# SEEDtk/genome.distance

Measured on AMD Instinct MI355X. Metric: genome-pair distances/sec (N×N), higher is better.
Workload: dtype u64; 1 GPU; c2: 1000 synthetic 2 Mbp genomes, DNA k=21 both strands, dictionary-rank bitsets; genomes=1000, genome_length=2000000, k=21, parallelism=rows1, dictionary_size=4000518, method=bitset

## Files before the change

### genome.distance_amd/csrc/gdist_api.hip

```cpp
#include <cstring>
#include <rocprim/rocprim.hpp>

#include <algorithm>
#include <thread>
#include <cmath>
#include <cstring>
#include <new>

#include "gdist_internal.hpp"
#include "group_stats_host.hpp"

namespace gdist {

const char* const kOptNames[OPT_COUNT] = {
#define GDIST_OPT_NAME(id, name) name,
    GDIST_OPTIONS(GDIST_OPT_NAME)
#undef GDIST_OPT_NAME
};

static int option_index(const char* name) {
    GD_REQUIRE(name != nullptr, "null option name");
    for (int i = 0; i < OPT_COUNT; i++)
        if (strcmp(kOptNames[i], name) == 0) return i;
    throw Error(GDIST_EINVAL, std::string("unknown option: ") + name);
// ... 725 lines not shown
int gdist_sets_rare_info(const gdist_sets* s, int64_t* threshold, int64_t* lists, int64_t* records) {
    return guard([&] {
        check_sets(s);
        if (threshold) *threshold = s->rare_T;
        if (lists) *lists = s->n_rare;
        if (records) *records = s->rare_records;
    });
}

int gdist_sets_sparse_info(const gdist_sets* s, int64_t* sparse_words, int64_t* dense_words, int64_t* entries) {
    return guard([&] {
        check_sets(s);
        if (sparse_words) *sparse_words = s->sparse ? s->Ws : 0;
        if (dense_words) *dense_words = s->sparse ? s->Wd : s->W;
        if (entries) *entries = s->sparse ? s->sp_entries : 0;
    });
}

int gdist_sets_variant_info(const gdist_sets* s, int64_t* kmers, int64_t* words, int64_t* entries, double* products) {
    return guard([&] {
        check_sets(s);
        if (kmers) *kmers = s->variant ? s->vw_kmers : 0;
        if (words) *words = s->variant ? s->vw_words : 0;
        if (entries) *entries = s->variant ? s->vw_entries : 0;
        if (products) *products = s->variant ? s->vw_products : 0.0;
    });
}

int gdist_sets_variant_layout(const gdist_sets* s, int* word_kmers, int* member_bytes, int64_t* row_weight_max) {
    return guard([&] {
// ... 1401 lines not shown
```

### genome.distance_amd/csrc/gdist_internal.hpp

```cpp
#pragma once

#include <hip/hip_runtime.h>
#include <rccl/rccl.h>

#include <algorithm>
#include <atomic>
#include <climits>
#include <functional>
#include <cstdint>
#include <map>
#include <memory>
#include <mutex>
#include <stdexcept>
#include <string>
#include <chrono>
#include <cstdio>
#include <cstdlib>
#include <vector>

#include "../../include/gdist.h"

namespace gdist {

struct Error : std::runtime_error {
// ... 143 lines not shown
    X(BITSET_DIAG, "bitset_diag")                        \
    X(BITSET_PARTIAL_RR, "bitset_partial_rr")     \
    X(BITSET_WG_PER_CU, "bitset_wg_per_cu")                                   \
    X(BITSET_MIN_CHUNKS, "bitset_min_chunks")      \
    X(REPS_BLOCK, "reps_block")                                \
    X(LOCUS_ORDER, "locus_order")                                            \
    X(SPARSE, "sparse")                                                                \
    X(SPARSE_ZMAX, "sparse_zmax")                    \
    X(SPARSE_WG_PER_CU, "sparse_wg_per_cu")               \
    X(SPARSE_SUN, "sparse_sun")                           \
    X(SPARSE_DYN, "sparse_dyn")                \
    X(SPARSE_BATCH, "sparse_batch")            \
    X(SPARSE_WTAIL, "sparse_wtail")            \
    X(SPARSE_DIAG22, "sparse_diag22")          \
    X(SPARSE_RPART22, "sparse_rpart22")        \
    X(SPARSE_MT, "sparse_mt")                    \
    X(SKETCH_K, "sketch_k")                                \
    X(SKETCH_TILE, "sketch_tile")                                         \
    X(SKETCH_V2, "sketch_v2")                              \
    X(SKETCH_PHASE, "sketch_phase")            \
    X(SKETCH_CAP, "sketch_cap")                          \
    X(SKETCH_RING, "sketch_ring")                              \
    X(SKETCH_WAIT, "sketch_wait")              \
    X(SPARSE_PART_BUDGET, "sparse_part_budget")        \
    X(GUIDES, "guides")                              \
    X(FORCE_EXCHANGE, "force_exchange")          \
    X(SPARSE_CHUNKS, "sparse_chunks")                         \
    X(GRAPH, "graph")                                      \
    X(TIME_KERNELS, "time_kernels")            \
    X(STEP_TIMING, "step_timing")                        \
    X(SPARSE_RARE, "sparse_rare")              \
// ... 158 lines not shown
    gdist::DevBuf post_w;
    gdist::DevBuf srare_w;
    gdist::DevBuf srare_skip;
    int64_t rare_kmers = 0;
    gdist::DevBuf guide_codes;
    gdist::DevBuf guide_keys;
    int64_t n_guide = 0;
    bool sparse = false;
    gdist::DevBuf dbits;
    gdist::DevBuf fp4;
    int64_t fp4_W = 0;
    int64_t Wd = 0;
    int64_t Ws = 0;
    gdist::DevBuf sp_off;
    gdist::DevBuf sp_ent;
    gdist::DevBuf sp_nc;
    int64_t sp_entries = 0, sp_U = 0;
    int64_t sp_pos_words = 0;
    bool sp_fold_dense = false;
    int sp_fold_slabs = 0;
    gdist::DevBuf sp_grp, sp_V, sp_T;
    int64_t sp_groups = 0, sp_group_words = 0;
    std::vector<int32_t> sp_bucket_bits;
    int64_t sp_nbk = 0;
    std::vector<double> sp_cost;
    std::vector<gdist::Summary> pack_sum;
    double sp_products = 0, sp_items = 0;
    double sp_pairs = 0;
    bool variant = false;
    int64_t vw_words = 0, vw_entries = 0, vw_kmers = 0, vw_dmin = 0, vw_max_list = 0;
// ... 410 lines not shown
```

### genome.distance_amd/csrc/sparse.hip

```cpp
#include <algorithm>
#include <map>
#include <cmath>
#include <cstring>

#include "gdist_internal.hpp"
#include "sparse_bounds.hpp"

namespace gdist {
namespace {

inline int grid_for(int64_t n, int block = 256, int64_t cap = 256 * 32) {
    int64_t g = ceil_div(n, block);
    return (int)std::max<int64_t>(1, std::min<int64_t>(g, cap));
}

constexpr int SB = 128;
constexpr int SNT = 512;
constexpr int kBucketShift = 10;

__global__ void locus_key_kernel(const uint64_t* __restrict__ gcodes, const uint64_t* __restrict__ gkeys, int64_t ng,
                                 const uint64_t* __restrict__ dict, int64_t U, uint64_t tag,
                                 uint64_t* __restrict__ key) {
    const int64_t stride = (int64_t)gridDim.x * blockDim.x;
    for (int64_t g = (int64_t)blockIdx.x * blockDim.x + threadIdx.x; g < ng; g += stride) {
// ... 293 lines not shown
    const int32_t* V = nullptr;
    const int32_t* T = nullptr;
    int m = 0;
    int64_t N = 0;
    __device__ __forceinline__ int at(int64_t i, int64_t j) const {
        if (!grp) return 0;
        const int gi = grp[i], gj = grp[j];
        int x = 0;
        if (gi >= 0) x += V[(int64_t)gi * N + j];
        if (gj >= 0) x += V[(int64_t)gj * N + i];
        if (gi >= 0 && gj >= 0) x += T[gi * m + gj];
        return x;
    }
};

__host__ __device__ __forceinline__ int cnt_index(int a, int b) {
    return ((a * 64 + ((b >> 1) ^ (a & 63))) << 1) | (b & 1);
}
__host__ __device__ __forceinline__ void cnt_pair(int t, int& a, int& b) {
    const int d = t >> 1;
    a = d >> 6;
    b = (((d & 63) ^ (a & 63)) << 1) | (t & 1);
}
__host__ __device__ __forceinline__ uint32_t row_code(int s) { return ((uint32_t)s << 8) | ((uint32_t)(s & 63) << 2); }
__host__ __device__ __forceinline__ uint32_t col_code(int s) {
    return ((uint32_t)(s & 1) << 4) | (((uint32_t)(s >> 1) << 2) << 16);
}
constexpr uint32_t kLastOfList = 32;
constexpr int kSentinelRecs = 512;
__device__ __forceinline__ void cnt_add(uint32_t* cnt, uint32_t r, uint32_t c, uint32_t v) {
    atomicAdd(reinterpret_cast<uint32_t*>(reinterpret_cast<char*>(cnt) + (r ^ (c >> 16))), v << (c & 31));
}

struct Rec3 {
    uint32_t a, b, c;
};
__device__ __forceinline__ unsigned long long rec_word(const ulonglong2& r) { return (r.x >> 32) | (r.y << 32); }
__device__ __forceinline__ uint32_t rec_row(const ulonglong2& r) { return (uint32_t)r.x; }
__device__ __forceinline__ uint32_t rec_col(const ulonglong2& r) { return (uint32_t)(r.y >> 32); }
__global__ void sparse_records_kernel(const unsigned long long* __restrict__ word, const uint8_t* __restrict__ set,
                                      int64_t n, ulonglong2* __restrict__ ent) {
    const int64_t stride = (int64_t)gridDim.x * blockDim.x;
    for (int64_t e = (int64_t)blockIdx.x * blockDim.x + threadIdx.x; e < n; e += stride) {
        const int st = set[e];
        const unsigned long long w = word[e];
        ent[e] = make_ulonglong2((unsigned long long)row_code(st) | (w << 32),
                                 (w >> 32) | ((unsigned long long)col_code(st) << 32));
    }
}

__global__ void sparse_last_kernel(const int64_t* __restrict__ off, int64_t nlists, ulonglong2* __restrict__ ent) {
    const int64_t stride = (int64_t)gridDim.x * blockDim.x;
    for (int64_t t = (int64_t)blockIdx.x * blockDim.x + threadIdx.x; t < nlists; t += stride) {
        const int64_t b = off[t], e = off[t + 1];
        if (e > b) ent[e - 1].y |= (unsigned long long)kLastOfList << 32;
    }
}

struct RareRows {
    const int64_t* soff = nullptr;
    const uint64_t* sent = nullptr;
    const uint32_t* sw = nullptr;
    const uint16_t* sskip = nullptr;
    const uint32_t* psets = nullptr;
};
inline RareRows rare_rows_of(const gdist_sets* s) {
    return RareRows{s->srare_off.as<int64_t>(), s->srare_ent.as<uint64_t>(), s->srare_w.as<uint32_t>(),
                    s->srare_skip.as<uint16_t>(), s->post_sets.as<uint32_t>()};
}

// ... 240 lines not shown
        const uint32_t v10 = (uint32_t)(__popc(a1[u].y & b0[u].y) + __popc(a1[u].z & b0[u].z)) & ne[u];
        const uint32_t v11 = (uint32_t)(__popc(a1[u].y & b1[u].y) + __popc(a1[u].z & b1[u].z)) & (ne[u] & lb);
        cnt_add(cnt, a0[u].x, b0[u].w, v00);
        cnt_add(cnt, a0[u].x, b1[u].w, v01);
        cnt_add(cnt, a1[u].x, b0[u].w, v10);
        cnt_add(cnt, a1[u].x, b1[u].w, v11);
        if (mirror) {
            cnt_add(cnt, b0[u].x, a0[u].w, v00);
            cnt_add(cnt, b1[u].x, a0[u].w, v01);
            cnt_add(cnt, b0[u].x, a1[u].w, v10);
            cnt_add(cnt, b1[u].x, a1[u].w, v11);
        }
    }
}

template <int SU, int MODE>
__device__ __forceinline__ void sparse_step(const int4* __restrict__ rec, const unsigned long long* __restrict__ masks,
                                            int W0, int last, int fb, int lane, const SparseWalk& e,
                                            uint32_t* __restrict__ cnt, bool mirror) {
    if (MODE == 0) sparse_diag_slots<SU>(rec, masks, W0, last, fb, lane, e, cnt, mirror);
    else if (MODE == 1) sparse_off_slots<SU>(rec, masks, W0, last, fb, lane, e, cnt);
    else if (MODE == 2) sparse_off22_slots<SU>(rec, masks, W0, last, fb, lane, e, cnt);
    else sparse_diag22_slots<SU>(rec, masks, W0, last, fb, lane, e, cnt, mirror);
}

template <int SUN, int MODE>
__device__ __forceinline__ void sparse_walk(const int4* __restrict__ rec, unsigned long long* __restrict__ masks,
                                            int last, int total, int lane, const SparseWalk& e,
                                            uint32_t* __restrict__ cnt, bool mirror, bool wtail) {
    constexpr int G = kWinGroups / SUN * SUN;
    for (int W0 = 0; W0 < total; W0 += 64 * G) {
        if (lane < G) masks[lane] = 0ull;
        __builtin_amdgcn_wave_barrier();
        __atomic_signal_fence(__ATOMIC_SEQ_CST);
        const uint32_t rel = (uint32_t)(last - W0);
        if (rel < 64u * G) atomicOr(&masks[rel >> 6], 1ull << (rel & 63));
        __builtin_amdgcn_wave_barrier();
// ... 11 lines not shown
        __atomic_signal_fence(__ATOMIC_SEQ_CST);
    }
}

struct TileWalk {
    const uint32_t* offA;
    const uint32_t* offB;
    const ulonglong2* ent;
    uint32_t ra0, cb0;
    uint32_t zA, zB;
    SparseWalk e;
    int rlo, rhi;
    bool rpart, diag, mirror, r22;
    bool d22;
    bool wtail;
};

template <int SUN, int MT>
__device__ __forceinline__ void global_batch(const TileWalk& tc, int64_t s0, int64_t be, int only, int lane,
                                             int4* __restrict__ wrec, unsigned long long* __restrict__ masks,
                                             uint32_t* __restrict__ cnt) {
    const uint32_t* offA = tc.offA;
    const uint32_t* offB = tc.offB;
    const ulonglong2* ent = tc.ent;
    const uint32_t ra0 = tc.ra0, cb0 = tc.cb0;
    const uint32_t zA = tc.zA, zB = tc.zB;
    const SparseWalk& e = tc.e;
    const int rlo = tc.rlo, rhi = tc.rhi;
    const bool rpart = tc.rpart, diag = tc.diag, mirror = tc.mirror, r22 = tc.r22;
    const bool d22 = MT == 2 && tc.d22;
    const bool wtail = tc.wtail;
    const int bn = be - s0 < kBatchWords ? (int)(be - s0) : kBatchWords;
    uint32_t rb = ra0, cb = cb0;
    if (lane <= bn) {
        rb = offA[2 * (s0 + lane)];
        cb = offB[2 * (s0 + lane)];
    }
    const uint32_t re = wave_next_lane(rb), ce = wave_next_lane(cb);
    int nr = 0, ncl = 0;
    if (lane < bn && (only < 0 || lane == only)) {
        nr = (int)(re - rb);
        ncl = (int)(ce - cb);
        if (rpart) {
            int a = 0, en = nr;
            for (int t = 0; t < nr; t++) {
                const int st = (int)((uint32_t)ent[(int64_t)rb + t].x >> 8);
                a += st < rlo;
                en -= st >= rhi;
            }
            rb += a;
            nr = en > a ? en - a : 0;
        }
    }
    const int ncd = diag ? ncl : (ncl + 1) >> 1;
    const int hp = (nr + 1) >> 1;
    const int P = diag ? (d22 ? (nr >= 2 ? hp * (hp + 1) / 2 : 0) : nr * (nr - 1) / 2)
                       : (r22 ? hp : nr) * ncd;
    const int incl = wave_scan_incl(P);
    const int total = __builtin_amdgcn_readlane(incl, 63);
    const unsigned long long nz = __ballot(P > 0);
    const int k = (int)__builtin_amdgcn_mbcnt_hi((uint32_t)(nz >> 32), __builtin_amdgcn_mbcnt_lo((uint32_t)nz, 0u));
    if (P > 0) {
        if (diag) {
            wrec[k] = make_int4(-(incl - P), (int32_t)(rb - ra0), 0, 0);
        } else {
            const uint32_t rcp = (uint32_t)__float_as_int(__builtin_amdgcn_rcpf(2.0f * (float)ncd));
            wrec[k] = make_int4(-2 * (incl - P), (int32_t)((rb - ra0) << 4), (int32_t)((cb - cb0) << 4),
                                (int32_t)((rcp & 0xFFFFFF00u) | (uint32_t)(2 * ncd)));
        }
    }
    if (lane == 0) {
        const int nw = __popcll(nz);
        wrec[nw] = diag ? make_int4(-total, (int32_t)zA, 0, 0)
                        : make_int4(-2 * total, (int32_t)(zA << 4), (int32_t)(zB << 4), 0);
    }
    const int last = P > 0 ? incl - 1 : 0x7FFFFFFF;
    __builtin_amdgcn_wave_barrier();
    __atomic_signal_fence(__ATOMIC_SEQ_CST);
    if (MT == 2 && diag && d22) sparse_walk<2, 3>(wrec, masks, last, total, lane, e, cnt, mirror, wtail);
    else if (diag) sparse_walk<SUN, 0>(wrec, masks, last, total, lane, e, cnt, mirror, wtail);
    else if (MT == 2 && r22) sparse_walk<MT == 2 ? SUN : 1, 2>(wrec, masks, last, total, lane, e, cnt, false, wtail);
    else sparse_walk<SUN, 1>(wrec, masks, last, total, lane, e, cnt, false, wtail);
}

template <int SUN, int MT>
__global__ __launch_bounds__(SNT, 8) void sparse_tile_kernel(
    const int64_t* __restrict__ off, const ulonglong2* __restrict__ ent, const int32_t* __restrict__ nc, int64_t Us,
    int64_t Ws, const int2* __restrict__ tiles, const int32_t* __restrict__ cbnd, const int4* __restrict__ tinfo,
    const int2* __restrict__ wgmap, int nchunks, int64_t r0, int64_t r1,
    int64_t c0, int64_t c1, int upper, int32_t* __restrict__ I, int64_t ldI, int32_t* __restrict__ part, int64_t Wdp,
    int64_t N, const unsigned long long* __restrict__ slab_bits, int slabs, GroupPart gp, int xmap, int ntiles,
    RareSlab rs, int dyn, int diag22, int rpart22, int batch, int wtail) {
    __shared__ __attribute__((aligned(16))) uint32_t cnt[SB * SB / 2];
    __shared__ int4 rec[SNW][64];
    int& next_batch = rec[0][63].w;
    const unsigned ntw = gridDim.x - (unsigned)rs.nrare;
    if (blockIdx.x >= ntw) {
        rare_slab_row(rs, (int)(blockIdx.x - ntw), r0, c0, c1, upper, cnt);
        return;
    }
    const unsigned bid = blockIdx.x;
    int tile, ch;
    if (wgmap) {
        const int2 m = wgmap[bid];
        tile = m.x;
        ch = m.y;
    } else if (xmap) {
// ... 9 lines not shown
    const int4 ti = tinfo[tile];
    cbnd += ti.x;
    const int rlo = (int)(r0 - A * SB > 0 ? r0 - A * SB : 0);
    const int rhi = (int)(r1 - A * SB < SB ? r1 - A * SB : SB);
    const bool rpart = rlo > 0 || (rhi < SB && r1 < N);
    const bool diag = A == B && !rpart, mirror = diag && !upper;
    const bool r22 = MT == 2 && !diag && (!rpart || rpart22);
    static_assert(SB * SB / 8 % SNT == 0, "whole 16-byte stores per thread");
#pragma unroll
    for (int t = 0; t < SB * SB / 8 / SNT; t++)
        reinterpret_cast<uint4*>(cnt)[t * SNT + threadIdx.x] = make_uint4(0, 0, 0, 0);
    if (threadIdx.x == 0) next_batch = SNW;
    __syncthreads();
    const int wv = __builtin_amdgcn_readfirstlane(threadIdx.x >> 6), lane = threadIdx.x & 63;
    const int64_t sb = cbnd[ch], se = cbnd[ch + 1];
    const int64_t* offA = off + A * Ws;
    const int64_t* offB = off + B * Ws;
    const int64_t ra0 = offA[sb], cb0 = offB[sb];
    const int64_t ntot = off[(int64_t)ceil_div(N, SB) * Ws];
    const uint32_t zA = (uint32_t)(ntot - ra0), zB = (uint32_t)(ntot - cb0);
    const TileWalk tc{reinterpret_cast<const uint32_t*>(offA), reinterpret_cast<const uint32_t*>(offB), ent,
                      (uint32_t)ra0, (uint32_t)cb0, zA, zB,
                      SparseWalk{reinterpret_cast<const char*>(ent + ra0), reinterpret_cast<const char*>(ent + cb0)},
                      rlo, rhi, rpart, diag, mirror, r22, diag22 != 0, wtail != 0};
    int4* wrec = &rec[wv][0];
    unsigned long long* masks = reinterpret_cast<unsigned long long*>(&rec[wv][kBatchWords + 1]);
    const int n = (int)(se - sb);
    int bw = batch > 0 ? batch : n <= SNW * kBatchWords ? (n + SNW - 1) / SNW : kBatchWords;
    bw = bw < 1 ? 1 : bw > kBatchWords ? kBatchWords : bw;
    const int64_t per = ceil_div(se - sb, (int64_t)SNW);
    const int64_t wb = dyn ? sb + (int64_t)wv * bw : sb + (int64_t)wv * per;
    const int64_t we = dyn ? se : (wb + per < se ? wb + per : se);
    for (int64_t s0 = wb; s0 < we;) {
        global_batch<SUN, MT>(tc, s0, s0 + bw < we ? s0 + bw : we, -1, lane, wrec, masks, cnt);
        if (dyn) {
            int nb = 0;
            if (lane == 0) nb = atomicAdd(&next_batch, 1);
            s0 = sb + (int64_t)__builtin_amdgcn_readfirstlane(nb) * bw;
        } else {
// ... 160 lines not shown
bool locus_order_enabled(const gdist_ctx* ctx) { return ctx->option(OPT_LOCUS_ORDER, 1) != 0; }

void free_sparse(gdist_sets* s) {
    if (s->ctx) {
        (void)hipStreamSynchronize(s->ctx->side);
        (void)hipStreamSynchronize(s->ctx->tile2);
        (void)hipStreamSynchronize(s->ctx->stream);
    }
    s->fp4.release();
    s->fp4_W = 0;
    s->graphs.clear();
    s->plans.clear();
    s->dbits.release();
    s->sp_off.release();
    s->sp_ent.release();
    s->sp_nc.release();
    s->sparse = false;
    s->Wd = s->Ws = s->sp_entries = s->sp_U = 0;
    s->sp_bucket_bits.clear();
    s->sp_nbk = 0;
    s->sp_cost.clear();
    s->sp_pos_words = 0;
    s->sp_fold_dense = false;
    s->sp_fold_slabs = 0;
    s->sp_products = s->sp_items = s->sp_pairs = 0.0;
    s->sp_grp.release();
    s->sp_V.release();
    s->sp_T.release();
    s->sp_groups = s->sp_group_words = 0;
}
// ... 241 lines not shown
        for (int64_t k = 0; k < Ws; k++) zs[k] = z[sw[k]];
        s->sp_cost = sparse_granule_costs(zs.data(), Ws);
    }
    GD_HIP(hipGetLastError());
    s->sp_ent.alloc((total + kSentinelRecs) * 16, st);
    GD_HIP(hipMemsetAsync(s->sp_ent.as<ulonglong2>() + total, 0, kSentinelRecs * 16, st));
    if (total) {
        sparse_records_kernel<<<grid_for(total), 256, 0, st>>>(sp_word.as<unsigned long long>(),
                                                                sp_set.as<uint8_t>(), total,
                                                                s->sp_ent.as<ulonglong2>());
        GD_HIP(hipGetLastError());
        sparse_last_kernel<<<grid_for(nblk * Ws), 256, 0, st>>>(s->sp_off.as<int64_t>(), nblk * Ws,
                                                                s->sp_ent.as<ulonglong2>());
    }
    GD_HIP(hipGetLastError());
    if (grouped) {
        DevBuf T((size_t)mg * mg * 4, st);
        GD_HIP(hipMemsetAsync(T.p, 0, (size_t)mg * mg * 4, st));
        group_t_kernel<<<(unsigned)grouped, 256, 0, st>>>(dpats.as<unsigned long long>(), grouped, mg,
                                                           T.as<int32_t>());
        GD_HIP(hipGetLastError());
        GD_HIP(hipStreamSynchronize(st));
        s->sp_grp = std::move(dgrp);
        s->sp_V = std::move(dV);
        s->sp_T = std::move(T);
        s->sp_groups = mg;
        s->sp_group_words = grouped;
    }
    if (Wdp) {
        DevBuf ddw(Wd * 4, st);
// ... 278 lines not shown
}

bool sparse_matrix(gdist_ctx* ctx, const gdist_sets* s, int64_t r0, int64_t r1, int64_t c0, int64_t c1, bool upper,
                   int32_t* d_I, int64_t ldI, hipStream_t st, SparseScratch& sc, const SparseEpilogue* ep,
                   const SparsePipe* pp) {
    if (!s->sparse || r1 <= r0 || c1 <= c0) return false;
    sparse_plan(ctx, s, r0, r1, c0, c1, upper, st, sc);
    GD_REQUIRE(!ep || (sc.use_part && (s->n_rare == 0 || sc.rare_in)), "fused sparse epilogue without its plan");
    GD_REQUIRE(!pp || (ep && sc.pipe), "pipelined sparse step without its buffer copies");
    if (sc.ntiles == 0) return false;
    hipStream_t tst = pp ? pp->tile_st : st;
    const DevBuf& part = pp && pp->copy ? sc.part2 : sc.part;
    const DevBuf& rare_slab = pp && pp->copy ? sc.rare_slab2 : sc.rare_slab;
    const int nchunks = sc.nchunks;
    const int64_t nt = sc.ntiles;
    const int mt = (int)ctx->option(OPT_SPARSE_MT, 2);
    const int sun = (int)ctx->option(OPT_SPARSE_SUN, mt == 2 ? 3 : 4);
    GD_REQUIRE(sun >= 2 && sun <= 4, "sparse_sun: 2, 3 or 4");
    GD_REQUIRE(mt == 1 || mt == 2, "sparse_mt: 1 (1 x 2 micro-tiles) or 2 (2 x 2)");
    const int batch = (int)ctx->option(OPT_SPARSE_BATCH, 0);
    GD_REQUIRE(batch >= 0 && batch <= kBatchWords, "sparse_batch: 0 (by the chunk) or 1..48 words");
    auto kern = mt == 2 ? (sun == 2 ? sparse_tile_kernel<2, 2> : sun == 4 ? sparse_tile_kernel<4, 2> : sparse_tile_kernel<3, 2>)
                        : (sun == 2 ? sparse_tile_kernel<2, 1> : sun == 4 ? sparse_tile_kernel<4, 1> : sparse_tile_kernel<3, 1>);
    const bool rare = sc.use_part && sc.rare_in;
    FamilyTimer ft(ctx, GDIST_KERNEL_SPARSE, tst);
    const bool xmap = ctx->option(OPT_SPARSE_XCD, 0) != 0;
    RareSlab rs;
    if (rare) {
        rs.rr = rare_rows_of(s);
        rs.nch = (int)ceil_div(c1 - c0, kRareChunkCols);
        const int64_t nrare = (r1 - r0) * rs.nch;
        GD_REQUIRE(nrare < (int64_t(1) << 30), "too many rare rows");
        rs.nrare = (int)nrare;
        rs.slab = rare_slab.as<uint32_t>();
        rs.tile_of = sc.rare_tile.as<int32_t>();
        rs.ab0 = sc.rare_ab0;
        rs.nbc = sc.rare_nbc;
    }
    const int64_t grid = (xmap ? ceil_div(nchunks, 8) * 8 * nt : sc.total_chunks) + rs.nrare;
    GD_REQUIRE(grid < (int64_t(1) << 31), "sparse grid too large");
    kern<<<(unsigned)grid, SNT, 0, tst>>>(s->sp_off.as<int64_t>(), s->sp_ent.as<ulonglong2>(), s->sp_nc.as<int32_t>(),
                                         s->sp_U, s->Ws, sc.tiles.as<int2>(), sc.bounds.as<int32_t>(),
                                         sc.tinfo.as<int4>(), sc.wgmap.as<int2>(), nchunks, r0, r1,
                                         c0, c1, upper ? 1 : 0, d_I, ldI, sc.use_part ? part.as<int32_t>() : nullptr,
                                         s->Wd, s->nsets, s->dbits.as<unsigned long long>(), s->sp_fold_slabs,
                                         group_part(s), xmap ? 1 : 0, (int)nt, rs,
                                         (int)ctx->option(OPT_SPARSE_DYN, 1), (int)ctx->option(OPT_SPARSE_DIAG22, 1),
                                         (int)ctx->option(OPT_SPARSE_RPART22, 1), batch,
                                         (int)ctx->option(OPT_SPARSE_WTAIL, 1));
    GD_HIP(hipGetLastError());
    ft.end();
    if (pp) {
        GD_HIP(hipEventRecord(pp->ev_tile, tst));
        GD_HIP(hipStreamWaitEvent(st, pp->ev_tile, 0));
    }
    if (sc.use_part) {
        sparse_reduce_kernel<<<(unsigned)(nt * (SB * SB / kReduceCnt / kReduceGroups)), 256, 0, st>>>(
            part.as<int32_t>(), sc.tinfo.as<int4>(), sc.tiles.as<int2>(), s->sp_nc.as<int32_t>(), s->sp_U, r0, r1,
            c0, c1,
            upper ? 1 : 0, d_I, ldI,
            rare ? rare_slab.as<uint32_t>() : nullptr, ep ? ep->D : nullptr, ep ? ep->ldD : 0,
            ep ? ep->off : nullptr, ep ? ep->empty_nan : 0, group_part(s));
        GD_HIP(hipGetLastError());
    }
// ... 5 lines not shown
```

### genome.distance_amd/gdist/_lib.py

```python
from __future__ import annotations

import ctypes as C
import os

import numpy as np

_HERE = os.path.dirname(os.path.abspath(__file__))
LIB_PATH = os.path.join(_HERE, "libgdist.so")

OK, EINVAL, ENOMEM, EDEVICE, ECOMM = 0, -1, -2, -3, -4
DNA, PROT, SKETCH = 0, 1, 2
STRAND_BOTH, STRAND_FWD, STRAND_CANON = 0x0, 0x1, 0x2
AMBIG_DEFAULT, AMBIG_SKIP, AMBIG_KEEP = 0x0, 0x4, 0x8
NO_CASE_FOLD = 0x10
UPPER_TRIANGLE, OUT_DEVICE, EMPTY_NAN, SKETCH_JACCARD = 0x100, 0x200, 0x400, 0x800
METHOD_AUTO, METHOD_SORTED, METHOD_BITSET = 0, 1, 2
BITSET_KEEP_SINGLETONS = 0x1
ALLGATHER_CONSUME = 0x1
QUERY_ALL, QUERY_ANY_LE, QUERY_ARGMIN = 0, 1, 2
CLOSEST_KEEP_SELF, CLOSEST_MAX_N = 0x1000, 512
GROUP_MAX_TYPES = 8
HIST_MAX_EDGES = 1023
UNIQUE_ID_BYTES = 128
OPTION_DEFAULT = -(1 << 63)
# ... 20 lines not shown

lib = _load()

_PKG = os.path.dirname(_HERE)
_REPO = os.path.dirname(_PKG)


def tree_source_hash() -> str:
    import glob
    import hashlib
    files = sorted(glob.glob(os.path.join(_PKG, "csrc", "*.hip")))
    files += [os.path.join(_PKG, "csrc", "gdist_internal.hpp"), os.path.join(_PKG, "csrc", "sparse_bounds.hpp"),
              os.path.join(_PKG, "csrc", "group_stats_host.hpp"), os.path.join(_PKG, "csrc", "cross_plan.hpp"),
              os.path.join(_PKG, "csrc", "sketch_cross_merge.hpp"), os.path.join(_PKG, "csrc", "sketch_wave_merge.hpp"),
              os.path.join(_PKG, "csrc", "pair_list.hpp"), os.path.join(_PKG, "csrc", "cross_cut.hpp"),
              os.path.join(_REPO, "include", "gdist.h")]
    h = hashlib.sha256()
    for f in files:
        with open(f, "rb") as fh:
            h.update(fh.read())
    return h.hexdigest()[:16]


def check_build() -> str:
    built = lib.gdist_source_hash().decode()
    tree = tree_source_hash()
    if built != tree:
        raise ImportError(f"libgdist.so is stale: built from sources {built}, this tree is {tree}; "
                          "rebuild with `make -C genome.distance_amd`")
    return built
# ... 34 lines not shown
    "gdist_sets_info": (C.c_int, [_setp, C.POINTER(C.c_int), C.POINTER(C.c_int), _i64p, _i64p]),
    "gdist_sets_sizes": (C.c_int, [_setp, _i64p]),
    "gdist_sets_download": (C.c_int, [_setp, _i64p, _u64p]),
    "gdist_sets_build_bitsets": (C.c_int, [_setp, _u32]),
    "gdist_sets_build_bitsets_ex": (C.c_int, [_setp, _u32, _i64]),
    "gdist_sets_release_codes": (C.c_int, [_setp]),
    "gdist_sets_build_timing": (C.c_int, [_setp, _dblp, _dblp, _dblp, C.POINTER(C.c_int)]),
    "gdist_sets_rare_info": (C.c_int, [_setp, _i64p, _i64p, _i64p]),
    "gdist_sets_rare_stats": (C.c_int, [_setp, _i64p, _i64p]),
    "gdist_sets_rare_kmers": (C.c_int, [_setp, _i64p]),
    "gdist_sets_sparse_info": (C.c_int, [_setp, _i64p, _i64p, _i64p]),
    "gdist_sets_variant_info": (C.c_int, [_setp, _i64p, _i64p, _i64p, _dblp]),
    "gdist_sets_variant_layout": (C.c_int, [_setp, C.POINTER(C.c_int), C.POINTER(C.c_int), _i64p]),
    "gdist_sets_group_info": (C.c_int, [_setp, _i64p, _i64p]),
    "gdist_sets_sparse_sides": (C.c_int, [_setp, _i64p, _i64p]),
    "gdist_sets_sparse_pairs": (C.c_int, [_setp, C.POINTER(C.c_double)]),
    "gdist_sets_bitset_info": (C.c_int, [_setp, _i64p, _i64p]),
    "gdist_sets_bitset_download": (C.c_int, [_setp, _u64p]),
    "gdist_sets_concat": (C.c_int, [_setp, _setp, C.POINTER(_setp)]),
    "gdist_sets_prepare": (C.c_int, [_ctxp, _setp, C.c_int, _dbl, C.POINTER(C.c_int), _dblp, _dblp]),
    "gdist_intersect_matrix": (C.c_int, [_ctxp, _setp, _i64, _i64, _i64, _i64, C.c_int, _u32, _vp, _vp, _i64]),
    "gdist_greedy_reps": (C.c_int, [_ctxp, _setp, C.c_int, _dbl, _i64p, _i32p, _i64p, _dblp, _i64p]),
    "gdist_row_query": (C.c_int, [_ctxp, _setp, _i64, _i64p, _i64, C.c_int, _dbl, _dblp, _i32p, _i64p, _dblp]),
    "gdist_sketch_build": (C.c_int, [_ctxp, _setp, C.c_int, C.POINTER(_setp)]),
    "gdist_sketch_upload": (C.c_int, [_ctxp, C.c_int, _i64, _i64p, _i32p, C.POINTER(_setp)]),
    "gdist_sketch_download": (C.c_int, [_setp, _i64p, _i32p]),
    "gdist_sketch_matrix": (C.c_int, [_ctxp, _setp, _i64, _i64, _i64, _i64, _u32, _vp, _vp, _i64]),
    "gdist_sketch_pairs": (C.c_int, [_ctxp, _setp, _setp, _i64, _i64p, _i64p, _u32, _i32p, _dblp]),
    "gdist_lsh_build": (C.c_int, [_ctxp, _setp, C.c_int, C.c_int, C.c_uint64, C.POINTER(C.c_void_p)]),
    "gdist_lsh_free": (C.c_int, [C.c_void_p]),
# ... 73 lines not shown
```

### genome.distance_amd/gdist/kmers.py

```python
from __future__ import annotations

import contextlib
import ctypes as C
import enum
import math
import os
import weakref
from typing import Iterable, Mapping, Sequence

import numpy as np

from . import _lib as L


def option_names() -> list[str]:
    names, i = [], 0
    while True:
        p = C.c_char_p()
        if L.lib.gdist_ctx_option_name(i, C.byref(p)) != L.OK:
            return names
        names.append(p.value.decode())
        i += 1


# ... 757 lines not shown
    def variant_layout(self) -> tuple[int, int, int]:
        wk, mb, rw = C.c_int(), C.c_int(), C.c_int64()
        L.check(L.lib.gdist_sets_variant_layout(self.h, C.byref(wk), C.byref(mb), C.byref(rw)))
        return wk.value, mb.value, rw.value

    def group_info(self) -> tuple[int, int]:
        g, w = C.c_int64(), C.c_int64()
        L.check(L.lib.gdist_sets_group_info(self.h, C.byref(g), C.byref(w)))
        return g.value, w.value

    def sparse_sides(self) -> tuple[int, int]:
        a, b = C.c_int64(), C.c_int64()
        L.check(L.lib.gdist_sets_sparse_sides(self.h, C.byref(a), C.byref(b)))
        return a.value, b.value

    def sparse_pairs(self) -> float:
        p = C.c_double()
        L.check(L.lib.gdist_sets_sparse_pairs(self.h, C.byref(p)))
        return p.value

    def rare_kmers(self) -> int:
        n = C.c_int64()
        L.check(L.lib.gdist_sets_rare_kmers(self.h, C.byref(n)))
        return n.value

    def rare_info(self) -> tuple[int, int, int]:
        t, n, r = C.c_int64(), C.c_int64(), C.c_int64()
        L.check(L.lib.gdist_sets_rare_info(self.h, C.byref(t), C.byref(n), C.byref(r)))
        return t.value, n.value, r.value

# ... 304 lines not shown
```

### include/gdist.h

```cpp
#ifndef GDIST_H
#define GDIST_H

#include <stdint.h>

#ifdef __cplusplus
extern "C" {
#endif

#define GDIST_ABI_VERSION 1

#define GDIST_OK        0
#define GDIST_EINVAL   -1
#define GDIST_ENOMEM   -2
#define GDIST_EDEVICE  -3
#define GDIST_ECOMM    -4

#define GDIST_DNA     0
#define GDIST_PROT    1
#define GDIST_SKETCH  2

#define GDIST_STRAND_BOTH   0x0u
#define GDIST_STRAND_FWD    0x1u
#define GDIST_STRAND_CANON  0x2u
#define GDIST_STRAND_MASK   0x3u
// ... 67 lines not shown
int  gdist_sets_build_bitsets(gdist_sets* sets, unsigned flags);
int  gdist_sets_build_bitsets_ex(gdist_sets* sets, unsigned flags, int64_t rare_threshold);
int  gdist_sets_release_codes(gdist_sets* sets);
int  gdist_sets_build_timing(const gdist_sets* sets, double* build_ms, double* split_ms, double* share_max_ms,
                             int* shares);
int  gdist_sets_rare_info(const gdist_sets* sets, int64_t* threshold, int64_t* lists, int64_t* records);
int  gdist_sets_rare_kmers(const gdist_sets* sets, int64_t* kmers);
int  gdist_sets_rare_stats(const gdist_sets* sets, int64_t* pair_incs, int64_t* max_list);
int  gdist_sets_bitset_info(const gdist_sets* sets, int64_t* dict_size, int64_t* words_per_set);
int  gdist_sets_sparse_info(const gdist_sets* sets, int64_t* sparse_words, int64_t* dense_words, int64_t* entries);
int  gdist_sets_variant_info(const gdist_sets* sets, int64_t* kmers, int64_t* words, int64_t* entries,
                             double* products);
int  gdist_sets_variant_layout(const gdist_sets* sets, int* word_kmers, int* member_bytes, int64_t* row_weight_max);
int  gdist_sets_sparse_sides(const gdist_sets* sets, int64_t* complement_words, int64_t* positive_words);
int  gdist_sets_sparse_pairs(const gdist_sets* sets, double* pairs);
int  gdist_sets_group_info(const gdist_sets* sets, int64_t* groups, int64_t* grouped_words);
int  gdist_sets_bitset_download(const gdist_sets* sets, uint64_t* bits);
int  gdist_sets_concat(const gdist_sets* a, const gdist_sets* b, gdist_sets** out);

int  gdist_sets_prepare(gdist_ctx* ctx, gdist_sets* sets, int method, double pairs, int* chosen,
                        double* cost_bitset_s, double* cost_sorted_s);
int  gdist_intersect_matrix(gdist_ctx* ctx, const gdist_sets* sets,
                            int64_t r0, int64_t r1, int64_t c0, int64_t c1,
                            int method, unsigned flags,
                            int32_t* I_out, double* D_out, int64_t ld);
int  gdist_ctx_step_info(gdist_ctx* ctx, int64_t out[4]);
int  gdist_greedy_reps(gdist_ctx* ctx, const gdist_sets* sets, int method, double max_dist,
                       const int64_t* tie_rank, int32_t* is_rep, int64_t* rep_of, double* rep_dist,
                       int64_t* nreps);
int  gdist_row_query(gdist_ctx* ctx, const gdist_sets* sets, int64_t q,
// ... 122 lines not shown
```

Baseline: 5.837 billion pairs/s.

## Add 3x3 triple-packed micro-tile walk for sparse off-diagonal tiles

Packs each sparse word list into 32-byte triples (three 64-bit words plus encoded row/column counter codes) and adds a 3x3 micro-tile walk mode that forms nine popcount products per pair of loaded records. This mode becomes the default for off-diagonal, non-row-partitioned tiles. The aim is more register reuse per byte loaded than the 2x2 walk, at the cost of an extra build pass, extra device memory and padding waste in lists whose length is not a multiple of three. Whether the benchmark's bitset method actually reaches the sparse path is unclear.

```diff
diff --git a/genome.distance_amd/csrc/gdist_api.hip b/genome.distance_amd/csrc/gdist_api.hip
--- a/genome.distance_amd/csrc/gdist_api.hip
+++ b/genome.distance_amd/csrc/gdist_api.hip
@@ -763,6 +763,16 @@
         if (sparse_words) *sparse_words = s->sparse ? s->Ws : 0;
         if (dense_words) *dense_words = s->sparse ? s->Wd : s->W;
         if (entries) *entries = s->sparse ? s->sp_entries : 0;
+    });
+}
+
+int gdist_sets_sparse_triples(const gdist_sets* s, int64_t* out) {
+    return guard([&] {
+        check_sets(s);
+        GD_REQUIRE(out, "null output");
+        const bool have = s->sparse && s->sp_tri.p;
+        out[0] = have ? s->sp_triples : 0;
+        for (int k = 0; k < 4; k++) out[1 + k] = have ? s->sp_tri_lists[k] : 0;
     });
 }
 
diff --git a/genome.distance_amd/csrc/gdist_internal.hpp b/genome.distance_amd/csrc/gdist_internal.hpp
--- a/genome.distance_amd/csrc/gdist_internal.hpp
+++ b/genome.distance_amd/csrc/gdist_internal.hpp
@@ -181,7 +181,7 @@
     X(SPARSE_WTAIL, "sparse_wtail")            \
     X(SPARSE_DIAG22, "sparse_diag22")          \
     X(SPARSE_RPART22, "sparse_rpart22")        \
-    X(SPARSE_MT, "sparse_mt")                    \
+    X(SPARSE_MT, "sparse_mt")                  \
     X(SKETCH_K, "sketch_k")                                \
     X(SKETCH_TILE, "sketch_tile")                                         \
     X(SKETCH_V2, "sketch_v2")                              \
@@ -370,6 +370,10 @@
     int64_t Ws = 0;
     gdist::DevBuf sp_off;
     gdist::DevBuf sp_ent;
+    gdist::DevBuf sp_toff;
+    gdist::DevBuf sp_tri;
+    int64_t sp_triples = 0;
+    int64_t sp_tri_lists[4] = {0, 0, 0, 0};
     gdist::DevBuf sp_nc;
     int64_t sp_entries = 0, sp_U = 0;
     int64_t sp_pos_words = 0;
diff --git a/genome.distance_amd/csrc/sparse.hip b/genome.distance_amd/csrc/sparse.hip
--- a/genome.distance_amd/csrc/sparse.hip
+++ b/genome.distance_amd/csrc/sparse.hip
@@ -5,6 +5,7 @@
 
 #include "gdist_internal.hpp"
 #include "sparse_bounds.hpp"
+#include "sparse_triple.hpp"
 
 namespace gdist {
 namespace {
@@ -331,20 +332,9 @@
     }
 };
 
-__host__ __device__ __forceinline__ int cnt_index(int a, int b) {
-    return ((a * 64 + ((b >> 1) ^ (a & 63))) << 1) | (b & 1);
-}
-__host__ __device__ __forceinline__ void cnt_pair(int t, int& a, int& b) {
-    const int d = t >> 1;
-    a = d >> 6;
-    b = (((d & 63) ^ (a & 63)) << 1) | (t & 1);
-}
-__host__ __device__ __forceinline__ uint32_t row_code(int s) { return ((uint32_t)s << 8) | ((uint32_t)(s & 63) << 2); }
-__host__ __device__ __forceinline__ uint32_t col_code(int s) {
-    return ((uint32_t)(s & 1) << 4) | (((uint32_t)(s >> 1) << 2) << 16);
-}
 constexpr uint32_t kLastOfList = 32;
 constexpr int kSentinelRecs = 512;
+constexpr int kSparseMtDefault = 3;
 __device__ __forceinline__ void cnt_add(uint32_t* cnt, uint32_t r, uint32_t c, uint32_t v) {
     atomicAdd(reinterpret_cast<uint32_t*>(reinterpret_cast<char*>(cnt) + (r ^ (c >> 16))), v << (c & 31));
 }
@@ -371,6 +361,40 @@
     for (int64_t t = (int64_t)blockIdx.x * blockDim.x + threadIdx.x; t < nlists; t += stride) {
         const int64_t b = off[t], e = off[t + 1];
         if (e > b) ent[e - 1].y |= (unsigned long long)kLastOfList << 32;
+    }
+}
+
+__global__ void sparse_triple_count_kernel(const int64_t* __restrict__ off, int64_t nlists,
+                                           int32_t* __restrict__ tcnt, unsigned long long* __restrict__ cls) {
+    const int64_t t = (int64_t)blockIdx.x * blockDim.x + threadIdx.x;
+    int c = -1;
+    if (t < nlists) {
+        const int n = (int)(off[t + 1] - off[t]);
+        tcnt[t] = (n + 2) / 3;
+        c = n == 0 ? 0 : n % 3 == 0 ? 3 : n % 3;
+    } else if (t == nlists) {
+        tcnt[t] = 0;
+    }
+    for (int k = 0; k < 4; k++) {
+        const unsigned long long m = __ballot(c == k);
+        if (m && (threadIdx.x & 63) == 0) atomicAdd(&cls[k], (unsigned long long)__popcll(m));
+    }
+}
+__global__ void sparse_triples_kernel(const int64_t* __restrict__ off, const int64_t* __restrict__ toff64,
+                                      int64_t nlists, const unsigned long long* __restrict__ word,
+                                      const uint8_t* __restrict__ set, uint32_t* __restrict__ toff,
+                                      uint4* __restrict__ tri) {
+    const int64_t t = (int64_t)blockIdx.x * blockDim.x + threadIdx.x;
+    if (t > nlists) return;
+    const int64_t tb = toff64[t];
+    toff[t] = (uint32_t)tb;
+    if (t == nlists) return;
+    const int64_t b = off[t];
+    const int n = (int)(off[t + 1] - b);
+    for (int j = 0; 3 * j < n; j++) {
+        const Triple r = triple_pack(word + b + 3 * j, set + b + 3 * j, n - 3 * j < 3 ? n - 3 * j : 3);
+        tri[2 * (tb + j)] = make_uint4(r.d[0], r.d[1], r.d[2], r.d[3]);
+        tri[2 * (tb + j) + 1] = make_uint4(r.d[4], r.d[5], r.d[6], r.d[7]);
     }
 }
 
@@ -641,6 +665,56 @@
     }
 }
 
+template <int SU>
+__device__ __forceinline__ void sparse_off33_slots(const int4* __restrict__ rec,
+                                                   const unsigned long long* __restrict__ masks, int W0, int last,
+                                                   int fb, int lane, const SparseWalk& e, uint32_t* __restrict__ cnt) {
+    int4 r[SU];
+    unsigned long long m[SU];
+    const unsigned long long* mk = masks + ((fb - W0) >> 6);
+#pragma unroll
+    for (int u = 0; u < SU; u++) m[u] = mk[u];
+#pragma unroll
+    for (int u = 0; u < SU; u++) r[u] = rec[slot_rec(last, fb + 64 * u, m[u])];
+    uint32_t ri[SU], ci[SU];
+#pragma unroll
+    for (int u = 0; u < SU; u++) {
+        const int q2 = 2 * (fb + 64 * u) + 2 * lane + r[u].x;
+        const float rcp = __int_as_float(r[u].w);
+        const int xc = (int)__builtin_fmaf((float)q2, rcp, rcp);
+        const int yc2 = q2 - (int)__umul24((uint32_t)xc, (uint32_t)r[u].w & 0xFFu);
+        ri[u] = (uint32_t)r[u].y + ((uint32_t)xc << 5);
+        ci[u] = (uint32_t)r[u].z + ((uint32_t)yc2 << 4);
+    }
+    uint4 a0[SU], a1[SU], b0[SU], b1[SU];
+#pragma unroll
+    for (int u = 0; u < SU; u++) {
+        const char* pa = e.eA + ri[u];
+        const char* pb = e.eB + ci[u];
+        a0[u] = *reinterpret_cast<const uint4*>(pa);
+        a1[u] = *reinterpret_cast<const uint4*>(pa + 16);
+        b0[u] = *reinterpret_cast<const uint4*>(pb);
+        b1[u] = *reinterpret_cast<const uint4*>(pb + 16);
+    }
+#pragma unroll
+    for (int u = 0; u < SU; u++) {
+        const uint32_t al[3] = {a0[u].x, a0[u].z, a1[u].x}, ah[3] = {a0[u].y, a0[u].w, a1[u].y};
+        const uint32_t bl[3] = {b0[u].x, b0[u].z, b1[u].x}, bh[3] = {b0[u].y, b0[u].w, b1[u].y};
+#pragma unroll
+        for (int y = 0; y < 3; y++) {
+            const uint32_t co = triple_coff(b1[u].z, b1[u].w, y), sh = triple_shift(b1[u].z, b1[u].w, y);
+#pragma unroll
+            for (int x = 0; x < 3; x++) {
+                const uint32_t v = (uint32_t)(__popc(al[x] & bl[y]) + __popc(ah[x] & bh[y]));
+                const uint32_t rc = triple_row(a1[u].z, a1[u].w, x);
+                if (v) atomicAdd(reinterpret_cast<uint32_t*>(reinterpret_cast<char*>(cnt) + (rc ^ co)), v << sh);
+            }
+        }
+    }
+}
+
+constexpr int kTripleSlots = 2;
+
 template <int SU, int MODE>
 __device__ __forceinline__ void sparse_step(const int4* __restrict__ rec, const unsigned long long* __restrict__ masks,
                                             int W0, int last, int fb, int lane, const SparseWalk& e,
@@ -648,6 +722,7 @@
     if (MODE == 0) sparse_diag_slots<SU>(rec, masks, W0, last, fb, lane, e, cnt, mirror);
     else if (MODE == 1) sparse_off_slots<SU>(rec, masks, W0, last, fb, lane, e, cnt);
     else if (MODE == 2) sparse_off22_slots<SU>(rec, masks, W0, last, fb, lane, e, cnt);
+    else if (MODE == 4) sparse_off33_slots<SU>(rec, masks, W0, last, fb, lane, e, cnt);
     else sparse_diag22_slots<SU>(rec, masks, W0, last, fb, lane, e, cnt, mirror);
 }
 
@@ -689,6 +764,7 @@
     bool rpart, diag, mirror, r22;
     bool d22;
     bool wtail;
+    bool t33;
 };
 
 template <int SUN, int MT>
@@ -705,11 +781,13 @@
     const bool rpart = tc.rpart, diag = tc.diag, mirror = tc.mirror, r22 = tc.r22;
     const bool d22 = MT == 2 && tc.d22;
     const bool wtail = tc.wtail;
+    const bool t33 = MT == 2 && tc.t33;
+    const int osh = t33 ? 0 : 1, rsh = t33 ? 5 : 4;
     const int bn = be - s0 < kBatchWords ? (int)(be - s0) : kBatchWords;
     uint32_t rb = ra0, cb = cb0;
     if (lane <= bn) {
-        rb = offA[2 * (s0 + lane)];
-        cb = offB[2 * (s0 + lane)];
+        rb = offA[(s0 + lane) << osh];
+        cb = offB[(s0 + lane) << osh];
     }
     const uint32_t re = wave_next_lane(rb), ce = wave_next_lane(cb);
     int nr = 0, ncl = 0;
@@ -727,10 +805,10 @@
             nr = en > a ? en - a : 0;
         }
     }
-    const int ncd = diag ? ncl : (ncl + 1) >> 1;
+    const int ncd = diag || t33 ? ncl : (ncl + 1) >> 1;
     const int hp = (nr + 1) >> 1;
     const int P = diag ? (d22 ? (nr >= 2 ? hp * (hp + 1) / 2 : 0) : nr * (nr - 1) / 2)
-                       : (r22 ? hp : nr) * ncd;
+                       : (r22 && !t33 ? hp : nr) * ncd;
     const int incl = wave_scan_incl(P);
     const int total = __builtin_amdgcn_readlane(incl, 63);
     const unsigned long long nz = __ballot(P > 0);
@@ -740,20 +818,21 @@
             wrec[k] = make_int4(-(incl - P), (int32_t)(rb - ra0), 0, 0);
         } else {
             const uint32_t rcp = (uint32_t)__float_as_int(__builtin_amdgcn_rcpf(2.0f * (float)ncd));
-            wrec[k] = make_int4(-2 * (incl - P), (int32_t)((rb - ra0) << 4), (int32_t)((cb - cb0) << 4),
+            wrec[k] = make_int4(-2 * (incl - P), (int32_t)((rb - ra0) << rsh), (int32_t)((cb - cb0) << rsh),
                                 (int32_t)((rcp & 0xFFFFFF00u) | (uint32_t)(2 * ncd)));
         }
     }
     if (lane == 0) {
         const int nw = __popcll(nz);
         wrec[nw] = diag ? make_int4(-total, (int32_t)zA, 0, 0)
-                        : make_int4(-2 * total, (int32_t)(zA << 4), (int32_t)(zB << 4), 0);
+                        : make_int4(-2 * total, (int32_t)(zA << rsh), (int32_t)(zB << rsh), 0);
     }
     const int last = P > 0 ? incl - 1 : 0x7FFFFFFF;
     __builtin_amdgcn_wave_barrier();
     __atomic_signal_fence(__ATOMIC_SEQ_CST);
     if (MT == 2 && diag && d22) sparse_walk<2, 3>(wrec, masks, last, total, lane, e, cnt, mirror, wtail);
     else if (diag) sparse_walk<SUN, 0>(wrec, masks, last, total, lane, e, cnt, mirror, wtail);
+    else if (MT == 2 && t33) sparse_walk<kTripleSlots, MT == 2 ? 4 : 1>(wrec, masks, last, total, lane, e, cnt, false, wtail);
     else if (MT == 2 && r22) sparse_walk<MT == 2 ? SUN : 1, 2>(wrec, masks, last, total, lane, e, cnt, false, wtail);
     else sparse_walk<SUN, 1>(wrec, masks, last, total, lane, e, cnt, false, wtail);
 }
@@ -765,7 +844,8 @@
     const int2* __restrict__ wgmap, int nchunks, int64_t r0, int64_t r1,
     int64_t c0, int64_t c1, int upper, int32_t* __restrict__ I, int64_t ldI, int32_t* __restrict__ part, int64_t Wdp,
     int64_t N, const unsigned long long* __restrict__ slab_bits, int slabs, GroupPart gp, int xmap, int ntiles,
-    RareSlab rs, int dyn, int diag22, int rpart22, int batch, int wtail) {
+    RareSlab rs, int dyn, int diag22, int rpart22, int batch, int wtail, const uint32_t* __restrict__ toff,
+    const uint4* __restrict__ tri) {
     __shared__ __attribute__((aligned(16))) uint32_t cnt[SB * SB / 2];
     __shared__ int4 rec[SNW][64];
     int& next_batch = rec[0][63].w;
@@ -805,15 +885,18 @@
     __syncthreads();
     const int wv = __builtin_amdgcn_readfirstlane(threadIdx.x >> 6), lane = threadIdx.x & 63;
     const int64_t sb = cbnd[ch], se = cbnd[ch + 1];
-    const int64_t* offA = off + A * Ws;
-    const int64_t* offB = off + B * Ws;
-    const int64_t ra0 = offA[sb], cb0 = offB[sb];
-    const int64_t ntot = off[(int64_t)ceil_div(N, SB) * Ws];
-    const uint32_t zA = (uint32_t)(ntot - ra0), zB = (uint32_t)(ntot - cb0);
-    const TileWalk tc{reinterpret_cast<const uint32_t*>(offA), reinterpret_cast<const uint32_t*>(offB), ent,
-                      (uint32_t)ra0, (uint32_t)cb0, zA, zB,
-                      SparseWalk{reinterpret_cast<const char*>(ent + ra0), reinterpret_cast<const char*>(ent + cb0)},
-                      rlo, rhi, rpart, diag, mirror, r22, diag22 != 0, wtail != 0};
+    const bool t33 = MT == 2 && toff && !diag && !rpart;
+    const uint32_t* offA = t33 ? toff + A * Ws : reinterpret_cast<const uint32_t*>(off + A * Ws);
+    const uint32_t* offB = t33 ? toff + B * Ws : reinterpret_cast<const uint32_t*>(off + B * Ws);
+    const int osh = t33 ? 0 : 1, rsh = t33 ? 5 : 4;
+    const uint32_t ra0 = offA[sb << osh], cb0 = offB[sb << osh];
+    const int64_t nlists = (int64_t)ceil_div(N, SB) * Ws;
+    const uint32_t ntot = t33 ? toff[nlists] : (uint32_t)off[nlists];
+    const uint32_t zA = ntot - ra0, zB = ntot - cb0;
+    const char* recs = t33 ? reinterpret_cast<const char*>(tri) : reinterpret_cast<const char*>(ent);
+    const TileWalk tc{offA, offB, ent, ra0, cb0, zA, zB,
+                      SparseWalk{recs + ((int64_t)ra0 << rsh), recs + ((int64_t)cb0 << rsh)},
+                      rlo, rhi, rpart, diag, mirror, r22, diag22 != 0, wtail != 0, t33};
     int4* wrec = &rec[wv][0];
     unsigned long long* masks = reinterpret_cast<unsigned long long*>(&rec[wv][kBatchWords + 1]);
     const int n = (int)(se - sb);
@@ -1004,6 +1087,10 @@
     s->dbits.release();
     s->sp_off.release();
     s->sp_ent.release();
+    s->sp_toff.release();
+    s->sp_tri.release();
+    s->sp_triples = 0;
+    for (int64_t& c : s->sp_tri_lists) c = 0;
     s->sp_nc.release();
     s->sparse = false;
     s->Wd = s->Ws = s->sp_entries = s->sp_U = 0;
@@ -1275,6 +1362,33 @@
                                                                 s->sp_ent.as<ulonglong2>());
     }
     GD_HIP(hipGetLastError());
+    {
+        const int64_t nl = nblk * Ws;
+        DevBuf tcnt((nl + 1) * 4, st), t64((nl + 1) * 8, st), cls(4 * 8, st);
+        GD_HIP(hipMemsetAsync(cls.p, 0, 4 * 8, st));
+        sparse_triple_count_kernel<<<(unsigned)ceil_div(nl + 1, 256), 256, 0, st>>>(
+            s->sp_off.as<int64_t>(), nl, tcnt.as<int32_t>(), cls.as<unsigned long long>());
+        GD_HIP(hipGetLastError());
+        exclusive_scan_i32_to_i64(ctx, tcnt.as<int32_t>(), t64.as<int64_t>(), (size_t)(nl + 1));
+        int64_t ntri = 0;
+        unsigned long long hc[4] = {0, 0, 0, 0};
+        d2h(&ntri, t64.as<int64_t>() + nl, 8, st);
+        d2h(hc, cls.p, 4 * 8, st);
+        if (ntri + kSentinelTriples < (int64_t(1) << 27)) {
+            s->sp_toff.alloc((nl + 1) * 4, st);
+            s->sp_tri.alloc((ntri + kSentinelTriples) * kTripleBytes, st);
+            GD_HIP(hipMemsetAsync(s->sp_tri.as<char>() + ntri * kTripleBytes, 0, kSentinelTriples * kTripleBytes, st));
+            sparse_triples_kernel<<<(unsigned)ceil_div(nl + 1, 256), 256, 0, st>>>(
+                s->sp_off.as<int64_t>(), t64.as<int64_t>(), nl, sp_word.as<unsigned long long>(),
+                sp_set.as<uint8_t>(), s->sp_toff.as<uint32_t>(), s->sp_tri.as<uint4>());
+            GD_HIP(hipGetLastError());
+            s->sp_triples = ntri;
+            for (int k = 0; k < 4; k++) s->sp_tri_lists[k] = (int64_t)hc[k];
+        } else if (ctx->trace()) {
+            fprintf(stderr, "gdist: %lld sparse triples exceed the 3 x 3 walk's 2^27: the 2 x 2 walk stays\n",
+                    (long long)ntri);
+        }
+    }
     if (grouped) {
         DevBuf T((size_t)mg * mg * 4, st);
         GD_HIP(hipMemsetAsync(T.p, 0, (size_t)mg * mg * 4, st));
@@ -1583,10 +1697,12 @@
     const DevBuf& rare_slab = pp && pp->copy ? sc.rare_slab2 : sc.rare_slab;
     const int nchunks = sc.nchunks;
     const int64_t nt = sc.ntiles;
-    const int mt = (int)ctx->option(OPT_SPARSE_MT, 2);
-    const int sun = (int)ctx->option(OPT_SPARSE_SUN, mt == 2 ? 3 : 4);
+    int mt = (int)ctx->option(OPT_SPARSE_MT, kSparseMtDefault);
+    const int sun = (int)ctx->option(OPT_SPARSE_SUN, mt >= 2 ? 3 : 4);
     GD_REQUIRE(sun >= 2 && sun <= 4, "sparse_sun: 2, 3 or 4");
-    GD_REQUIRE(mt == 1 || mt == 2, "sparse_mt: 1 (1 x 2 micro-tiles) or 2 (2 x 2)");
+    GD_REQUIRE(mt >= 1 && mt <= 3, "sparse_mt: 1 (1 x 2 micro-tiles), 2 (2 x 2) or 3 (3 x 3 over triples)");
+    const bool t33 = mt == 3 && s->sp_tri.p;
+    if (mt == 3) mt = 2;
     const int batch = (int)ctx->option(OPT_SPARSE_BATCH, 0);
     GD_REQUIRE(batch >= 0 && batch <= kBatchWords, "sparse_batch: 0 (by the chunk) or 1..48 words");
     auto kern = mt == 2 ? (sun == 2 ? sparse_tile_kernel<2, 2> : sun == 4 ? sparse_tile_kernel<4, 2> : sparse_tile_kernel<3, 2>)
@@ -1616,7 +1732,9 @@
                                          group_part(s), xmap ? 1 : 0, (int)nt, rs,
                                          (int)ctx->option(OPT_SPARSE_DYN, 1), (int)ctx->option(OPT_SPARSE_DIAG22, 1),
                                          (int)ctx->option(OPT_SPARSE_RPART22, 1), batch,
-                                         (int)ctx->option(OPT_SPARSE_WTAIL, 1));
+                                         (int)ctx->option(OPT_SPARSE_WTAIL, 1),
+                                         t33 ? s->sp_toff.as<uint32_t>() : nullptr,
+                                         t33 ? s->sp_tri.as<uint4>() : nullptr);
     GD_HIP(hipGetLastError());
     ft.end();
     if (pp) {
diff --git a/genome.distance_amd/csrc/sparse_triple.hpp b/genome.distance_amd/csrc/sparse_triple.hpp
--- /dev/null
+++ b/genome.distance_amd/csrc/sparse_triple.hpp
@@ -0,0 +1,52 @@
+#pragma once
+
+#include <cstdint>
+
+#if defined(__HIPCC__)
+#define GDIST_ST_HD __host__ __device__ __forceinline__
+#else
+#define GDIST_ST_HD inline
+#endif
+
+namespace gdist {
+
+GDIST_ST_HD int cnt_index(int a, int b) { return ((a * 64 + ((b >> 1) ^ (a & 63))) << 1) | (b & 1); }
+GDIST_ST_HD void cnt_pair(int t, int& a, int& b) {
+    const int d = t >> 1;
+    a = d >> 6;
+    b = (((d & 63) ^ (a & 63)) << 1) | (t & 1);
+}
+GDIST_ST_HD uint32_t row_code(int s) { return ((uint32_t)s << 8) | ((uint32_t)(s & 63) << 2); }
+GDIST_ST_HD uint32_t col_code(int s) { return ((uint32_t)(s & 1) << 4) | (((uint32_t)(s >> 1) << 2) << 16); }
+
+struct Triple {
+    uint32_t d[8];
+};
+GDIST_ST_HD Triple triple_pack(const unsigned long long* w, const uint8_t* set, int n) {
+    Triple t;
+    int s[3];
+    for (int k = 0; k < 3; k++) {
+        const unsigned long long x = k < n ? w[k] : 0ull;
+        s[k] = k < n ? (int)set[k] : 0;
+        t.d[2 * k] = (uint32_t)x;
+        t.d[2 * k + 1] = (uint32_t)(x >> 32);
+    }
+    t.d[6] = row_code(s[0]) | (row_code(s[1]) << 16);
+    t.d[7] = row_code(s[2]) | ((uint32_t)(s[0] >> 1) << 18) | ((uint32_t)(s[1] >> 1) << 26);
+    return t;
+}
+GDIST_ST_HD uint32_t triple_row(uint32_t d6, uint32_t d7, int k) {
+    return k == 0 ? d6 & 0xFFFFu : k == 1 ? d6 >> 16 : d7 & 0xFFFFu;
+}
+GDIST_ST_HD uint32_t triple_coff(uint32_t d6, uint32_t d7, int k) {
+    (void)d6;
+    return k == 0 ? (d7 >> 16) & 0xFFu : k == 1 ? d7 >> 24 : (d7 >> 7) & 0xFCu;
+}
+GDIST_ST_HD uint32_t triple_shift(uint32_t d6, uint32_t d7, int k) {
+    return ((k == 0 ? d6 >> 4 : k == 1 ? d6 >> 20 : d7 >> 4)) & 16u;
+}
+
+constexpr int kTripleBytes = 32;
+constexpr int kSentinelTriples = 512;
+
+}
diff --git a/genome.distance_amd/gdist/_lib.py b/genome.distance_amd/gdist/_lib.py
--- a/genome.distance_amd/gdist/_lib.py
+++ b/genome.distance_amd/gdist/_lib.py
@@ -58,6 +58,7 @@
               os.path.join(_PKG, "csrc", "group_stats_host.hpp"), os.path.join(_PKG, "csrc", "cross_plan.hpp"),
               os.path.join(_PKG, "csrc", "sketch_cross_merge.hpp"), os.path.join(_PKG, "csrc", "sketch_wave_merge.hpp"),
               os.path.join(_PKG, "csrc", "pair_list.hpp"), os.path.join(_PKG, "csrc", "cross_cut.hpp"),
+              os.path.join(_PKG, "csrc", "sparse_triple.hpp"),
               os.path.join(_REPO, "include", "gdist.h")]
     h = hashlib.sha256()
     for f in files:
@@ -122,6 +123,7 @@
     "gdist_sets_variant_layout": (C.c_int, [_setp, C.POINTER(C.c_int), C.POINTER(C.c_int), _i64p]),
     "gdist_sets_group_info": (C.c_int, [_setp, _i64p, _i64p]),
     "gdist_sets_sparse_sides": (C.c_int, [_setp, _i64p, _i64p]),
+    "gdist_sets_sparse_triples": (C.c_int, [_setp, _i64p]),
     "gdist_sets_sparse_pairs": (C.c_int, [_setp, C.POINTER(C.c_double)]),
     "gdist_sets_bitset_info": (C.c_int, [_setp, _i64p, _i64p]),
     "gdist_sets_bitset_download": (C.c_int, [_setp, _u64p]),
diff --git a/genome.distance_amd/gdist/kmers.py b/genome.distance_amd/gdist/kmers.py
--- a/genome.distance_amd/gdist/kmers.py
+++ b/genome.distance_amd/gdist/kmers.py
@@ -795,6 +795,11 @@
         L.check(L.lib.gdist_sets_sparse_sides(self.h, C.byref(a), C.byref(b)))
         return a.value, b.value
 
+    def sparse_triples(self) -> tuple[int, int, int, int, int]:
+        out = (C.c_int64 * 5)()
+        L.check(L.lib.gdist_sets_sparse_triples(self.h, out))
+        return tuple(int(v) for v in out)
+
     def sparse_pairs(self) -> float:
         p = C.c_double()
         L.check(L.lib.gdist_sets_sparse_pairs(self.h, C.byref(p)))
diff --git a/include/gdist.h b/include/gdist.h
--- a/include/gdist.h
+++ b/include/gdist.h
@@ -105,6 +105,7 @@
 int  gdist_sets_variant_layout(const gdist_sets* sets, int* word_kmers, int* member_bytes, int64_t* row_weight_max);
 int  gdist_sets_sparse_sides(const gdist_sets* sets, int64_t* complement_words, int64_t* positive_words);
 int  gdist_sets_sparse_pairs(const gdist_sets* sets, double* pairs);
+int  gdist_sets_sparse_triples(const gdist_sets* sets, int64_t* out);
 int  gdist_sets_group_info(const gdist_sets* sets, int64_t* groups, int64_t* grouped_words);
 int  gdist_sets_bitset_download(const gdist_sets* sets, uint64_t* bits);
 int  gdist_sets_concat(const gdist_sets* a, const gdist_sets* b, gdist_sets** out);
```

New measurement: 6.830 billion pairs/s (median of 6 runs). 1.17x the previous value.
